# sleep3r/Diffusion-Handwriting-Generation.pytorch

Measured on AMD Instinct MI355X. Metric: stroke-points/sec reverse-sampled (T=60, L=488), higher is better.
Workload: dtype bf16; 1 GPU; configs[1]: batch=64 prompts/GPU, T=60, L=488, Lt=30, d_model=128/192/256, num_layers=2, diffusion_mode=new, random-init weights; global_batch=64, seq_len=488, parallelism=batch-shard x1 (no collectives)

## Files before the change

diffusion-handwriting-generation.pytorch_amd/csrc/attn_core.h:

```cpp
#pragma once
#include "dhw_common.h"

DHW_DEV void frag_keep_keys(Frag<bf16_t>& f, int n0, int n1) {
#pragma unroll
  for (int i = 0; i < 4; ++i) {
    f.v[i] = i < n0 ? f.v[i] : (bf16_t)0.0f;
    f.v[4 + i] = i < n1 ? f.v[4 + i] : (bf16_t)0.0f;
  }
}
DHW_DEV void frag_keep_keys(Frag<float>& f, int n0, int n1) {
#pragma unroll
  for (int i = 0; i < 4; ++i) {
    f.lo[i] = i < n0 ? f.lo[i] : 0.f;
    f.hi[i] = i < n1 ? f.hi[i] : 0.f;
  }
}
template <typename T, int D, int KB>
DHW_DEV void attn_wave16(const Frag<T> (&qf)[(D + 31) / 32], const T* krow, int ldk, const T* vrow, int lpad,
                         const int64_t* trow, int Lk, f32x4 (&o)[D / 16]) {
  constexpr int DT = D / 16, KCH = (D + 31) / 32, NTILE = KB / 16, NPF = KB / 32;
  const int lane = threadIdx.x & 63, g = lane >> 4;
  const float scale = rsqrtf((float)D);
  float m_run = -INFINITY, l_run = 0.f;
#pragma unroll
// ... 126 lines not shown
      const float e = __expf(s[t][r] - m_new);
      s[t][r] = e;
      psum += e;
    }
  l_run = l_run * alpha + psum;
  m_run = m_new;
  Frag<T> pf[NPF];
#pragma unroll
  for (int pp = 0; pp < NPF; ++pp) frag_from_f32(pf[pp], s[2 * pp], s[2 * pp + 1]);
#pragma unroll
  for (int t = 0; t < DT; ++t) {
    o[t] = o[t] * alpha;
#pragma unroll
    for (int pp = 0; pp < NPF; ++pp) {
      const T* vp = reinterpret_cast<const T*>(vt + (16 * t) * SV) + 32 * pp;
      mma32(o[t], frag_load_halves(vp, vp + 16), pf[pp]);
    }
  }
}

typedef __bf16 bf16x4_lds __attribute__((ext_vector_type(4)));
DHW_DEV Frag<bf16_t> frag_load_tr(const char* p0, const char* p1) {
  const bf16x4 a = __builtin_amdgcn_ds_read_tr16_b64_v4bf16((__attribute__((address_space(3))) bf16x4_lds*)(uintptr_t)p0);
  const bf16x4 b = __builtin_amdgcn_ds_read_tr16_b64_v4bf16((__attribute__((address_space(3))) bf16x4_lds*)(uintptr_t)p1);
  Frag<bf16_t> f;
  f.v = __builtin_shufflevector(a, b, 0, 1, 2, 3, 4, 5, 6, 7);
  return f;
}
template <typename T> DHW_DEV void vt_store_piece(char* row, int part, const uint4& v) {
  static_assert(sizeof(T) == 4, "bf16 kernels keep V row-major");
  *reinterpret_cast<uint4*>(row + part * 16) = v;
}

template <int D, int KB, bool MASKED, int NU, bool TAIL>
DHW_DEV void attn_block_bf16(int lane, const Frag<bf16_t> (*qf)[(D + 31) / 32], const char* const (&kt)[NU], int SK, const char* const (&vt)[NU], int SV, int kb,
                             unsigned padbits, int Lk, float (&m_run)[NU], float (&l_run)[NU], f32x4 (*o)[D / 16]) {
#pragma clang fp contract(off)
  typedef bf16_t T;
  constexpr int DT = D / 16, KCH = (D + 31) / 32, NTILE = KB / 16, NPF = KB / 32;
  static_assert(D % 32 == 0, "head width");
  const int g = lane >> 4;
  const float c = rsqrtf((float)D) * 1.4426950408889634f;
  f32x4 s[NU][NTILE];
  {
    Frag<T> kf[NU][NTILE][KCH];
    auto request = [&](int u) {
#pragma unroll
      for (int t = 0; t < NTILE; ++t)
#pragma unroll
        for (int ch = 0; ch < KCH; ++ch) kf[u][t][ch] = frag_load(reinterpret_cast<const T*>(kt[u] + t * 16 * SK) + 32 * ch + 8 * g);
    };
    auto multiply = [&](int u) {
#pragma unroll
      for (int t = 0; t < NTILE; ++t) {
        s[u][t] = (f32x4){0, 0, 0, 0};
#pragma unroll
        for (int ch = 0; ch < KCH; ++ch) mma32(s[u][t], kf[u][t][ch], qf[u][ch]);
      }
    };
    request(0);
#pragma unroll
    for (int u = 0; u < NU; ++u) {
      if (u + 1 < NU) request(u + 1);
      __builtin_amdgcn_sched_barrier(0);
      multiply(u);
      __builtin_amdgcn_sched_barrier(0);
    }
  }
#pragma unroll
  for (int u = 0; u < NU; ++u)
#pragma unroll
    for (int t = 0; t < NTILE; ++t) s[u][t] = s[u][t] * c;
  if constexpr (TAIL) {
#pragma unroll
    for (int u = 0; u < NU; ++u)
#pragma unroll
      for (int t = 0; t < NTILE; ++t)
#pragma unroll
        for (int r = 0; r < 4; ++r) s[u][t][r] = kb + 16 * t + 4 * g + r < Lk ? s[u][t][r] : -INFINITY;
  }
  if constexpr (MASKED) {
    const float neg = -1e9f * 1.4426950408889634f;
#pragma unroll
    for (int u = 0; u < NU; ++u)
#pragma unroll
      for (int t = 0; t < NTILE; ++t)
#pragma unroll
        for (int r = 0; r < 4; ++r) s[u][t][r] += ((padbits >> (4 * t + r)) & 1u) ? neg : 0.f;
  }
  Frag<T> vf[NU][DT][NPF];
#pragma unroll
  for (int u = 0; u < NU; ++u)
#pragma unroll
    for (int t = 0; t < DT; ++t)
#pragma unroll
      for (int pp = 0; pp < NPF; ++pp)
        vf[u][t][pp] = frag_load_tr(vt[u] + 32 * t + (32 * pp) * SV, vt[u] + 32 * t + (32 * pp + 16) * SV);
  __builtin_amdgcn_sched_barrier(0);
  float m_new[NU], alpha[NU];
#pragma unroll
  for (int u = 0; u < NU; ++u) {
    float mx = fmaxf(fmaxf(s[u][0][0], s[u][0][1]), fmaxf(s[u][0][2], s[u][0][3]));
#pragma unroll
    for (int t = 1; t < NTILE; ++t) mx = fmaxf(fmaxf(mx, fmaxf(s[u][t][0], s[u][t][1])), fmaxf(s[u][t][2], s[u][t][3]));
    m_new[u] = fmaxf(m_run[u], xg_max(mx));
    alpha[u] = __builtin_amdgcn_exp2f(m_run[u] - m_new[u]);
    m_run[u] = m_new[u];
  }
  Frag<T> pf[NU][NPF];
#pragma unroll
  for (int u = 0; u < NU; ++u) {
    const f32x4 negm = (f32x4){-m_new[u], -m_new[u], -m_new[u], -m_new[u]};
    f32x4 psum = (f32x4){0, 0, 0, 0};
#pragma unroll
    for (int t = 0; t < NTILE; ++t) {
      s[u][t] = s[u][t] - m_new[u];
#pragma unroll
      for (int r = 0; r < 4; ++r) s[u][t][r] = __builtin_amdgcn_exp2f(s[u][t][r]);
      psum += s[u][t];
    }
    l_run[u] = __builtin_fmaf(l_run[u], alpha[u], (psum[0] + psum[1]) + (psum[2] + psum[3]));
#pragma unroll
    for (int pp = 0; pp < NPF; ++pp) frag_from_f32(pf[u][pp], s[u][2 * pp], s[u][2 * pp + 1]);
  }
  if (kb != 0) {
#pragma unroll
    for (int u = 0; u < NU; ++u)
#pragma unroll
      for (int t = 0; t < DT; ++t) o[u][t] = o[u][t] * alpha[u];
  }
#pragma unroll
  for (int u = 0; u < NU; ++u)
#pragma unroll
    for (int t = 0; t < DT; ++t)
#pragma unroll
      for (int pp = 0; pp < NPF; ++pp) mma32(o[u][t], vf[u][t][pp], pf[u][pp]);
}
template <typename T, int KB, bool MASKED, int UMAX>
DHW_DEV void attn_units(int lane, const Frag<T> (&qf)[UMAX][2], const char* kt, int SK, const char* vt, int SV, int hs, int HS, int H, int kb,
                        unsigned padbits, int Lk, float (&mr)[UMAX], float (&lr)[UMAX], f32x4 (&o)[UMAX][4]) {
  constexpr int ES = sizeof(T);
  const int l15 = lane & 15, g = lane >> 4;
  const char* kt0 = kt + l15 * SK;
  if constexpr (sizeof(T) == 2) {
    const char* vt0 = vt + (4 * g + (l15 >> 2)) * SV + 4 * (l15 & 3) * ES;
#pragma unroll
    for (int u = 0; u < UMAX; ++u) {
      const int h = hs + u * HS;
      if (h < H) {
        const char* const ktu[1] = {kt0 + h * 64 * ES};
        const char* const vtu[1] = {vt0 + h * 64 * ES};
        float m1[1] = {mr[u]}, l1[1] = {lr[u]};
        if (kb + KB > Lk) attn_block_bf16<64, KB, MASKED, 1, true>(lane, qf + u, ktu, SK, vtu, SV, kb, padbits, Lk, m1, l1, o + u);
        else attn_block_bf16<64, KB, MASKED, 1, false>(lane, qf + u, ktu, SK, vtu, SV, kb, padbits, Lk, m1, l1, o + u);
        mr[u] = m1[0]; lr[u] = l1[0];
      }
    }
  } else {
    const char* vt0 = vt + l15 * SV;
#pragma unroll
    for (int u = 0; u < UMAX; ++u) {
      const int h = hs + u * HS;
      if (h < H) attn_block_lds<T, 64, KB>(lane, qf[u], kt0 + h * 64 * ES, SK, vt0 + h * 64 * SV + 4 * g * ES, SV, kb, padbits, Lk, mr[u], lr[u], o[u]);
    }
  }
}

template <int KB>
struct PadMask {
  int64_t tok[KB / 4];
  DHW_DEV void load(int lane, const int64_t* trow, int kb, int Lk) {
    const int g = lane >> 4;
    if (!trow) {
#pragma unroll
      for (int i = 0; i < KB / 4; ++i) tok[i] = 1;
      return;
    }
#pragma unroll
    for (int t = 0; t < KB / 16; ++t)
#pragma unroll
      for (int r = 0; r < 4; ++r) {
        const int key = kb + 16 * t + 4 * g + r;
        tok[4 * t + r] = trow[key < Lk ? key : Lk - 1];
      }
  }
  template <bool LAZY = false>
  DHW_DEV unsigned bits() const {
    unsigned m = 0;
#pragma unroll
    for (int i = 0; i < KB / 4; ++i) {
      int64_t t = tok[i];
      if constexpr (LAZY) asm volatile("" : "+v"(t));
      m |= (t == 0 ? 1u : 0u) << i;
    }
    return m;
  }
// ... 42 lines not shown
```

diffusion-handwriting-generation.pytorch_amd/csrc/enc_a_core.h:

```cpp
#pragma once
#include "attn_core.h"
#include "gemm_core.h"
#include "dhw_kernels.h"

#define ENC_STAMP(slot) do { DHW_STAMP_IF(p.stamps && blockIdx.x == 0 && threadIdx.x == 0, slot, __builtin_amdgcn_s_memrealtime()); \
                             DHW_STAMP_IF(p.stamps && (p.dbg & 4) && blockIdx.x == 0 && (threadIdx.x & 63) == 0, 64 + (threadIdx.x >> 6) * 32 + (slot), __builtin_amdgcn_s_memtime()); } while (0)

template <typename T, int BM>
DHW_DEV void stage_rows(char* dst, int S, const T* src, int C, int b, int L, int m0, int tid, int nthreads) {
  constexpr int ES = sizeof(T);
  const int cpr = C * ES / 16;
  const int total = BM * cpr;
  constexpr int U = 4;
  for (int base = tid; base < total; base += nthreads * U) {
    uint4 v[U];
    int off[U];
#pragma unroll
    for (int u = 0; u < U; ++u) {
      const int id = base + u * nthreads;
      const int r = id / cpr, cc = id - r * cpr;
      v[u] = make_uint4(0, 0, 0, 0);
      off[u] = id < total ? r * S + cc * 16 : -1;
      if (id < total && m0 + r < L)
        v[u] = *reinterpret_cast<const uint4*>(reinterpret_cast<const char*>(src) + ((size_t)(b * L + m0 + r) * C) * ES + (size_t)cc * 16);
    }
#pragma unroll
    for (int u = 0; u < U; ++u)
      if (off[u] >= 0) *reinterpret_cast<uint4*>(dst + off[u]) = v[u];
  }
}

template <int NT>
struct EpiParams {
  f32x4 bias[NT], gam[NT], bet[NT];
  DHW_DEV void load(const float* b, const float* g, const float* be, int n0) {
#pragma unroll
// ... 75 lines not shown
template <typename T, int DM> constexpr int qkv_stride() { return sizeof(T) == 2 ? 3 * DM : 2 * DM; }

template <int DM> constexpr int enc_wn() { return DM % 128 == 0 ? 8 : 6; }

template <typename T, int DM, int BM, int VPIECE = 16, typename P>
DHW_DEV void enc_a_body(const P& p, const EncALds& m, int b, int m0, int rows_valid) {
  constexpr int ES = sizeof(T);
  constexpr int WN = enc_wn<DM>(), WM = 1;
  constexpr int MT = BM / WM / 16, NT = DM / WN / 16, H = DM / 64, KC = DM / 32;
  static_assert(NT * WN * 16 == DM, "channel tiles must divide over the waves");
  const int tid = body_tid(), lane = tid & 63, wave = tid >> 6;
  const int l15 = lane & 15, g = lane >> 4;
  const bool act = WN * WM == 8 || wave < WN * WM;
  const int wm = act ? wave / WN : 0, wn = act ? wave % WN : 0;
  const int S = tile_stride<T>(DM);
  const int Ls = sample_len(p.lens, p.lsh, b, p.Lk);
  char* XR = m.XR;
  char* QR = m.QR;
  float* red = m.red;
  const float* gam = p.film + (size_t)b * p.film_bs;
  const float* bet = gam + p.film_tot;
  const int row0 = wm * (BM / WM), ntile0 = wn * NT;
  const int n0 = ntile0 * 16 + 4 * g;
  const size_t wlane = ((size_t)ntile0 * KC * 64 + lane) * 8;
  const char* xop = XR + (row0 + l15) * S + g * 8 * ES;
  const char* qop = QR + (row0 + l15) * S + g * 8 * ES;

  constexpr int RINGA = sizeof(T) == 4 ? 12 : 24;
  typedef WRing<T, NT, RINGA, (RINGA + NT - 1) / NT> RingT;
  RingT ring;
  constexpr bool SPREADA = sizeof(T) == 2;
  constexpr bool SPREADQ = sizeof(T) == 2 && MT > 1;
  constexpr int FCHA = RingT::template fill_chunks<KC>(), FQA = (FCHA + 3) / 4;
  EpiParams<NT> ep;
  ENC_STAMP(0);
  constexpr bool VROW = sizeof(T) == 2;
  constexpr int KBC = 32, SKC = tile_stride<T>(DM), SVC = VROW ? SKC : KBC * ES + OPAD<T>;
  constexpr int EPV = 16 / ES, CPR = DM / EPV, PPR = KBC / EPV;
  constexpr int UX = (BM * CPR + 511) / 512, UK = (KBC * CPR + 511) / 512, UV = VROW ? UK : (DM * PPR + 511) / 512;
  constexpr int QKS = qkv_stride<T, DM>();
  char* KT = m.KT;
  char* VT = m.VT;
  const T* k1s = reinterpret_cast<const T*>(p.k1) + (size_t)b * p.Lt * DM;
  const T* v1s = reinterpret_cast<const T*>(p.vt1) + (VROW ? (size_t)b * p.Lt * DM : (size_t)b * DM * p.lpadT);
  constexpr bool PLDS = enc_plds<T>();
  const float* PL = m.PL;
  const int64_t* trow = p.text ? p.text + (size_t)b * p.Lt : nullptr;
  PadMask<KBC> pad;
  struct KVRegs { CopyRegs<UK> ck; CopyRegs<UV> cv; };
  auto kv_store = [&](KVRegs& kv) {
    CopyRegs<UK>& ck = kv.ck;
    CopyRegs<UV>& cv = kv.cv;
    ck.store(KBC * CPR, tid, 512, [&](int id) { const int r = id / CPR, cc = id - r * CPR; return reinterpret_cast<uint4*>(KT + r * SKC + cc * 16); },
             [&](int id) { return id / CPR < p.Lt; });
    if constexpr (VROW)
      cv.store(KBC * CPR, tid, 512, [&](int id) { const int r = id / CPR, cc = id - r * CPR; return reinterpret_cast<uint4*>(VT + r * SVC + cc * 16); },
               [&](int id) { return id / CPR < p.Lt; });
    else
      cv.store_to(DM * PPR, tid, 512, [&](int id, const uint4& v) { const int ch = id / PPR, part = id - ch * PPR; vt_store_piece<T>(VT + ch * SVC, part, v); },
                  [&](int id) { return (id % PPR + 1) * EPV <= p.lpadT; });
  };
  {
    KVRegs kv_now;
    KVRegs& kv = [&]() -> KVRegs& { return kv_now; }();
    CopyRegs<UK>& ck = kv.ck;
    CopyRegs<UV>& cv = kv.cv;
// ... 74 lines not shown
      if (kb) {
        attn_stage_kv<T, KBC>(KT, SK, VT, SV, k1s, DM, v1s, VROW ? DM : p.lpadT, DM, kb, p.Lt, tid, 512);
        lds_barrier();
      }
      attn_units<T, KBC, true, UMAX>(lane, qf, KT, SK, VT, SV, hs, HS, H, kb, padbits, p.Lt, mr, lr, o);
      if (kb + KBC < p.Lt) lds_barrier();
    }
#pragma unroll
    for (int u = 0; u < UMAX; ++u) {
      const int h = hs + u * HS;
      float l = lr[u];
      l = xg_sum(l);
      const float inv = 1.0f / l;
      if (h < H) {
        T* dst = reinterpret_cast<T*>(QR + (rg * 16 + l15) * S) + h * 64 + 4 * g;
        store_pair(lane, dst, dst + 16, o[u][0] * inv, o[u][1] * inv);
        store_pair(lane, dst + 32, dst + 48, o[u][2] * inv, o[u][3] * inv);
      }
    }
  }
  if (act) {
    ring.template fill_s<KC>(reinterpret_cast<const T*>(p.w_d1) + wlane);
    if constexpr (!PLDS) ep.load(p.b_d1, gam + p.f1, bet + p.f1, n0);
  }
  lds_barrier();
  ENC_STAMP(3);

  {
    f32x4 acc[NT][MT];
    acc_zero(acc);
    if (act) {
      ring.template run_s<MT, KC>(acc, qop, S, KC);
      ENC_STAMP(10);
      if constexpr (SPREADA) { ring.template fill_begin<KC>(reinterpret_cast<const T*>(p.w_qkv2) + wlane); ring.template fill_range<KC, 0, FQA>(); }
      else ring.template fill_s<KC>(reinterpret_cast<const T*>(p.w_qkv2) + wlane);
      if constexpr (PLDS) ep.lds(PL + DM, PL + 2 * DM, PL + 3 * DM, n0);
#pragma unroll
      for (int i = 0; i < NT; ++i)
#pragma unroll
        for (int j = 0; j < MT; ++j) acc[i][j] += ep.bias[i];
      if constexpr (SPREADA) ring.template fill_range<KC, FQA, 2 * FQA>();
    }
    if constexpr (SPREADA) ln_rows<T, MT, NT, WN, BM>(acc, red, wn, row0, lane, DM, act, [&]() { if (act) ring.template fill_range<KC, 2 * FQA, 3 * FQA>(); });
    else ln_rows<T, MT, NT, WN, BM>(acc, red, wn, row0, lane, DM, act);
    if constexpr (SPREADA) { if (act) ring.template fill_range<KC, 3 * FQA, FCHA>(); }
    ENC_STAMP(11);
    if (act) {
#pragma unroll
      for (int i = 0; i < NT; ++i)
#pragma unroll
        for (int j = 0; j < MT; ++j)
          acc[i][j] = acc[i][j] * ep.gam[i] + ep.bet[i] + load4(reinterpret_cast<const T*>(XR + (row0 + j * 16 + l15) * S) + n0 + 16 * i);
      enc_store_tiles<T, NT, MT>(lane, XR, S, row0, n0, acc);
    }
  }
  lds_barrier();
  ENC_STAMP(4);
  tile_copy_out<T>(XR, S, reinterpret_cast<T*>(p.x2) + (size_t)(b * p.Lk + m0) * DM, DM, rows_valid, DM, tid, 512, DHW_STORE_OF(p.store_a, 1));

  auto qkv_chunk = [&](auto CHUNK_) __attribute__((always_inline)) {
    constexpr int chunk = decltype(CHUNK_)::value;
    int opaque = 0;
    asm volatile("" : "+v"(opaque));
    f32x4 acc[NT][MT];
    acc_zero(acc);
    f32x4 pb[NT][MT];
    const bool rows_out = chunk < 2 || VROW;
    if (act) {
      if constexpr (!PLDS) ep.load_bias(p.b_qkv2 + chunk * DM, n0 + opaque);
      if (chunk < 2) {
#pragma unroll
        for (int i = 0; i < NT; ++i)
#pragma unroll
          for (int j = 0; j < MT; ++j)
            pb[i][j] = *reinterpret_cast<const f32x4*>(p.pb_qk2 + (unsigned)((m0 + row0 + j * 16 + l15) * 2 * DM + chunk * DM + n0 + 16 * i + opaque));
      } else {
#pragma unroll
        for (int i = 0; i < NT; ++i)
#pragma unroll
          for (int j = 0; j < MT; ++j) pb[i][j] = (f32x4){0, 0, 0, 0};
      }
      ring.template run_s<MT, KC>(acc, xop + opaque, S, KC);
      ENC_STAMP(12 + chunk);
      if constexpr (PLDS) ep.lds_bias(PL + (4 + chunk) * DM, n0 + opaque);
      if constexpr (SPREADA && MT == 1) {
        if (chunk < 2) { ring.template fill_begin<KC>(reinterpret_cast<const T*>(p.w_qkv2) + (size_t)(chunk + 1) * DM * DM + wlane); ring.template fill_range<KC, 0, 2 * FQA>(); }
      } else if constexpr (SPREADQ) {
        if (chunk < 2) { ring.template fill_begin<KC>(reinterpret_cast<const T*>(p.w_qkv2) + (size_t)(chunk + 1) * DM * DM + wlane); ring.template fill_range<KC, 0, FQA>(); }
      } else { if (chunk < 2) ring.template fill_s<KC>(reinterpret_cast<const T*>(p.w_qkv2) + (size_t)(chunk + 1) * DM * DM + wlane); }
    }
    if (rows_out && MT == 1) {
      const int r = row0 + l15;
      if (act && r < rows_valid) {
#pragma unroll
        for (int i = 0; i < NT; ++i)
          store4(reinterpret_cast<T*>(p.qk2) + (unsigned)((b * p.Lk + m0 + r) * QKS + chunk * DM + n0 + 16 * i + opaque), acc[i][0] + ep.bias[i] + pb[i][0]);
      }
      if constexpr (SPREADA && MT == 1) { if (act && chunk < 2) ring.template fill_range<KC, 2 * FQA, FCHA>(); }
      ENC_STAMP(5 + chunk);
      return;
    }
    constexpr bool QALT = sizeof(T) == 2;
    char* const QT = QALT && chunk == 1 ? m.KT : QR;
    static_assert(!QALT || (size_t)BM * tile_stride<T>(DM) <= enc_a_text_kv_bytes<T, DM, BM>(), "a staging tile inside the text K / V tiles");
    if constexpr (!QALT) lds_barrier();
    if (rows_out) {
      if (act) {
#pragma unroll
        for (int i = 0; i < NT; ++i)
#pragma unroll
          for (int j = 0; j < MT; ++j) acc[i][j] += ep.bias[i] + pb[i][j];
        if constexpr (SPREADQ) { if (chunk < 2) ring.template fill_range<KC, FQA, 2 * FQA>(); }
        enc_store_tiles<T, NT, MT>(lane, QT, S, row0, n0 + opaque, acc);
        if constexpr (SPREADQ) { if (chunk < 2) ring.template fill_range<KC, 2 * FQA, 3 * FQA>(); }
      }
      lds_barrier();
      tile_copy_out<T>(QT, S, reinterpret_cast<T*>(p.qk2) + (size_t)(b * p.Lk + m0) * QKS + chunk * DM, QKS, rows_valid, DM, tid, 512, DHW_STORE_OF(p.store_a, 1));
      if constexpr (SPREADQ) { if (act && chunk < 2) ring.template fill_range<KC, 3 * FQA, FCHA>(); }
    } else if constexpr (!VROW) {
      constexpr int SV = BM * ES + 16;
      char* VS = m.VS;
      if (act) {
#pragma unroll
        for (int i = 0; i < NT; ++i)
#pragma unroll
          for (int j = 0; j < MT; ++j) {
            const int rl = row0 + j * 16 + l15;
            const f32x4 v = acc[i][j] + ep.bias[i];
#pragma unroll
            for (int k = 0; k < 4; ++k)
              *reinterpret_cast<T*>(VS + (n0 + 16 * i + k) * SV + rl * ES) = from_f<T>(rl < rows_valid ? v[k] : 0.f);
          }
      }
      lds_barrier();
      constexpr int KPP = VPIECE / ES, PPR = BM / KPP;
      const int klimit = m0 + rows_valid >= Ls ? min(BM, p.lpadX - m0) : rows_valid;
      for (int id = tid; id < DM * PPR; id += 512) {
        const int ch = id / PPR, part = id - ch * PPR;
        if ((part + 1) * KPP <= klimit) {
          T* dst = reinterpret_cast<T*>(p.vt2) + ((size_t)b * DM + ch) * p.lpadX + m0 + part * KPP;
          const char* src = VS + ch * SV + part * VPIECE;
          if constexpr (VPIECE == 16) *reinterpret_cast<uint4*>(dst) = *reinterpret_cast<const uint4*>(src);
          else *reinterpret_cast<uint32_t*>(dst) = *reinterpret_cast<const uint32_t*>(src);
        }
      }
    }
    ENC_STAMP(5 + chunk);
  };
  qkv_chunk(std::integral_constant<int, 0>{});
  qkv_chunk(std::integral_constant<int, 1>{});
  qkv_chunk(std::integral_constant<int, 2>{});
// ... 3 lines not shown
```

diffusion-handwriting-generation.pytorch_amd/csrc/enc_bc_core.h:

```cpp
#pragma once
#include "enc_a_core.h"

namespace {

#define STAMP(slot) ENC_STAMP(slot)
#ifdef DHW_STAMPS
#define WST(slot) do { if (p.stamps && blockIdx.x == 0 && lane == 0) p.stamps[64 + wave * 32 + (slot)] = __builtin_amdgcn_s_memtime(); } while (0)
#else
#define WST(slot) do { } while (0)
#endif

template <typename T, int DM, int BM, typename P>
DHW_DEV void enc_a_tile(const P& p, const int b, const int m0, char* smem) {
  const int S = tile_stride<T>(DM);
  EncALds m;
  m.XR = smem;
  m.QR = m.XR + BM * S;
  m.red = reinterpret_cast<float*>(m.QR + BM * S);
  m.KT = reinterpret_cast<char*>(m.red) + 2 * 8 * BM * sizeof(float);
  m.VT = m.KT + 32 * tile_stride<T>(DM);
  m.VS = smem;
  m.PL = reinterpret_cast<float*>(m.KT + enc_a_text_kv_bytes<T, DM, BM>());
  const int Ls = sample_len(p.lens, p.lsh, b, p.Lk);
  if constexpr (DHW_LENS) { if (m0 >= Ls) return; }
  enc_a_body<T, DM, BM>(p, m, b, m0, min(BM, Ls - m0));
}

template <typename T, int DM, int BM>
constexpr size_t self_att_bytes(int kbs, int nbuf, int vpad = 16) {
  return (size_t)BM * tile_stride<T>(DM) + nbuf * ((size_t)kbs * tile_stride<T>(DM) + (sizeof(T) == 2 ? (size_t)kbs * tile_stride<T>(DM) : (size_t)DM * (kbs * sizeof(T) + vpad)));
}
template <typename T, int DM, int BM>
constexpr int self_kbs() { return sizeof(T) == 2 ? 64 : 32; }
template <typename T, int DM, int BM>
// ... 45 lines not shown
  const int row0 = wm * (BM / WM), ntile0 = wn * NT;
  const int n0 = ntile0 * 16 + 4 * g;
  const size_t wlane = ((size_t)ntile0 * KC * 64 + lane) * 8;
  const char* op1 = R1 + (row0 + l15) * S + g * 8 * ES;
  const char* op3 = R3 + (row0 + l15) * S + g * 8 * ES;

  WRing<T, NT, RING, RDMAX> ring;
  constexpr bool SPREAD = sizeof(T) == 2;
  constexpr int FCH = WRing<T, NT, RING, RDMAX>::template fill_chunks<KC>(), FQ = (FCH + 3) / 4;
  EpiParams<NT> ep;
  constexpr bool PLDS = enc_plds<T>(), PLFIX = bc_params_fixed<T, DM, BM>();
  float* PL = reinterpret_cast<float*>(smem + lds_bc_tiles<T, DM, BM>());
  ParamStage<8> cp;
#define BC_PARAMS_REQUEST() cp.template load<DM>(tid, p.b_d2, gam + p.f2, bet + p.f2, p.b_f1, p.b_f1 + DM, p.b_f2, gam + p.f3, bet + p.f3)
  STAMP(16);
  WST(0);
  DHW_STAMP_IF(p.stamps && blockIdx.x == 0 && threadIdx.x == 0, 40, __builtin_amdgcn_s_memtime());
  if (!(p.dbg & 1)) {
    constexpr int RG = BM / 16, HS = 8 / RG, UMAX = (H + HS - 1) / HS, KBS = self_kbs<T, DM, BM>();
    constexpr bool DB = self_db<T, DM, BM>();
    constexpr bool VROW = sizeof(T) == 2;
    constexpr int SK = tile_stride<T>(DM), SV = VROW ? SK : KBS * ES + self_vpad<T, DM, BM>();
    constexpr int BUFB = KBS * SK + (VROW ? KBS * SV : DM * SV);
    constexpr int QKS = qkv_stride<T, DM>();
    const int rg = wave % RG, hs = wave / RG;
    auto unit_head = [&](int u) { return hs + u * HS; };
    const T* qk = reinterpret_cast<const T*>(p.qk2);
    const T* ksrc = qk + (size_t)b * p.Lk * QKS + DM;
    const T* vsrc = VROW ? ksrc + DM : reinterpret_cast<const T*>(p.vt2) + (size_t)b * DM * p.lpadX;
    constexpr int EPV = 16 / ES, CPR = DM / EPV, PPR = KBS / EPV;
    constexpr int UK = (KBS * CPR + 511) / 512, UV = VROW ? UK : (DM * PPR + 511) / 512;
    CopyRegs<UK> ck;
    CopyRegs<UV> cv;
    auto request = [&](int kb) {
      ck.load(KBS * CPR, tid, 512, [&](int id) { const int r = id / CPR, cc = id - r * CPR;
                                                 return reinterpret_cast<const uint4*>(ksrc + (size_t)min(kb + r, p.Lk - 1) * QKS + cc * EPV); });
      if constexpr (VROW)
        cv.load(KBS * CPR, tid, 512, [&](int id) { const int r = id / CPR, cc = id - r * CPR;
                                                   return reinterpret_cast<const uint4*>(vsrc + (size_t)min(kb + r, p.Lk - 1) * QKS + cc * EPV); });
      else
        cv.load(DM * PPR, tid, 512, [&](int id) { const int ch = id / PPR, part = id - ch * PPR;
                                                  return reinterpret_cast<const uint4*>(vsrc + (size_t)ch * p.lpadX + (kb + (part + 1) * EPV <= p.lpadX ? kb + part * EPV : 0)); });
    };
    auto commit = [&](int kb, char* KT, char* VT) {
      ck.store(KBS * CPR, tid, 512, [&](int id) { const int r = id / CPR, cc = id - r * CPR; return reinterpret_cast<uint4*>(KT + r * SK + cc * 16); },
               [&](int id) { return kb + id / CPR < Ls; });
      if constexpr (VROW)
        cv.store(KBS * CPR, tid, 512, [&](int id) { const int r = id / CPR, cc = id - r * CPR; return reinterpret_cast<uint4*>(VT + r * SV + cc * 16); },
                 [&](int id) { return kb + id / CPR < Ls; });
      else
        cv.store_to(DM * PPR, tid, 512, [&](int id, const uint4& v) { const int ch = id / PPR, part = id - ch * PPR; vt_store_piece<T>(VT + ch * SV, part, v); },
                    [&](int id) { return kb + (id % PPR + 1) * EPV <= p.lpadX && (!DHW_LENS || kb + (id % PPR) * EPV < Ls); });
    };
    Frag<T> qf[UMAX][2];
    float mr[UMAX], lr[UMAX];
    f32x4 o[UMAX][4];
#pragma unroll
    for (int u = 0; u < UMAX; ++u) {
      const int h = unit_head(u);
      const T* qrow = qk + (size_t)(b * p.Lk + m0 + rg * 16 + l15) * QKS + (h < H ? h : 0) * 64 + 8 * g;
      qf[u][0] = frag_load(qrow);
      qf[u][1] = frag_load(qrow + 32);
      mr[u] = -INFINITY;
      lr[u] = 0.f;
#pragma unroll
      for (int t = 0; t < 4; ++t) o[u][t] = (f32x4){0, 0, 0, 0};
    }
    if constexpr (PLDS) BC_PARAMS_REQUEST();
    request(0);
    if constexpr (PLDS && PLFIX) cp.template store<DM>(PL, tid);
    commit(0, R2, R2 + KBS * SK);
    lds_barrier();
    int ib = 0;
    auto key_block = [&](int kb) {
      const bool more = kb + KBS < Ls;
      char* KT = R2 + (DB && (ib & 1) ? BUFB : 0);
      char* VT = KT + KBS * SK;
      char* KN = R2 + (DB && !(ib & 1) ? BUFB : 0);
      if (DB && more) request(kb + KBS);
      if (ib < 3) STAMP(26 + 2 * ib);
      attn_units<T, KBS, false, UMAX>(lane, qf, KT, SK, VT, SV, hs, HS, H, kb, 0u, Ls, mr, lr, o);
      if (ib < 3) STAMP(27 + 2 * ib);
      if (more) {
        if (!DB) {
          lds_barrier();
          request(kb + KBS);
        }
        commit(kb + KBS, KN, KN + KBS * SK);
        lds_barrier();
      }
    };
    for (int kb = 0; kb < Ls; kb += KBS, ++ib) key_block(kb);
    if constexpr (PLDS && !PLFIX) {
      static_assert(DB, "a single staging buffer leaves room for a fixed parameter block");
      static_assert((size_t)2 * BM * tile_stride<T>(DM) + 2 * 8 * BM * sizeof(float) + enc_bc_param_bytes<T, DM>() <= (size_t)BUFB, "parameter block inside buffer 0");
      PL = reinterpret_cast<float*>(((ib - 1) & 1) ? R2 + 2 * BM * S + 2 * 8 * BM * sizeof(float) : R2 + BUFB);
      cp.template store<DM>(PL, tid);
    }
    WST(1);
#pragma unroll
    for (int u = 0; u < UMAX; ++u) {
      const int h = unit_head(u);
      float l = lr[u];
      l = xg_sum(l);
      const float inv = 1.0f / l;
      if (h < H) {
        T* dst = reinterpret_cast<T*>(R1 + (rg * 16 + l15) * S) + h * 64 + 4 * g;
        store_pair(lane, dst, dst + 16, o[u][0] * inv, o[u][1] * inv);
        store_pair(lane, dst + 32, dst + 48, o[u][2] * inv, o[u][3] * inv);
      }
    }
  }
  else if constexpr (PLDS) {
    BC_PARAMS_REQUEST();
    if constexpr (!PLFIX) PL = reinterpret_cast<float*>(R2 + 2 * BM * S + 2 * 8 * BM * sizeof(float));
    cp.template store<DM>(PL, tid);
  }
  if (act) {
    ring.template fill_s<KC>(reinterpret_cast<const T*>(p.w_d2) + wlane);
    if constexpr (!PLDS) ep.load(p.b_d2, gam + p.f2, bet + p.f2, n0);
  }
  WST(2);
  lds_barrier();
  WST(3);
  STAMP(17);
// ... 171 lines not shown
```

diffusion-handwriting-generation.pytorch_amd/csrc/gemm_core.h:

```cpp
#pragma once
#include "dhw_common.h"
#include "dhw_kernels.h"
#include "epilogue.h"

template <typename T> constexpr int OPAD = sizeof(T) == 2 ? 32 : 16;
template <typename T> __host__ __device__ constexpr int tile_stride(int C) { return C * (int)sizeof(T) + OPAD<T>; }

DHW_DEV void keep_alive(const Frag<bf16_t>& f) { asm volatile("" ::"v"(f.v)); }
DHW_DEV void keep_alive(const Frag<float>& f) { asm volatile("" ::"v"(f.lo), "v"(f.hi)); }

#ifndef DHW_ABL
#define DHW_ABL 0
#endif
template <typename T, int NT, int RING = (sizeof(T) == 2 ? 24 : 12), int DMAX = 8>
struct WRing {
  static constexpr int D0 = RING / NT;
  static constexpr int D = D0 < 2 ? 2 : (D0 > DMAX ? DMAX : D0);
  Frag<T> q[D][NT];
  const T* base;
  int KT, KTS;

  DHW_DEV void fill(const T* __restrict__ wbase, int kt, int kts = 0) {
    base = wbase;
    KT = kt;
// ... 186 lines not shown
    for (int s = 0; s < KT_; ++s) {
      if (s + PF < KT_) request((s + PF) % NB);
      __builtin_amdgcn_sched_barrier(0);
#pragma unroll
      for (int i = 0; i < NT; ++i)
#pragma unroll
        for (int j = 0; j < MT; ++j) mma32(acc[i][j], q[s][i], a[s % NB][j]);
      if (s < DN) next_chunk(s);
#pragma unroll
      for (int e = 0; e < PER; ++e)
        if (KT_ + s * PER + e < DN) next_chunk(KT_ + s * PER + e);
      __builtin_amdgcn_sched_barrier(0);
    }
    base = nbase; KT = KTN_; KTS = nKTS;
  }
};

template <typename T, int MT, int NT, int RING = (sizeof(T) == 2 ? 24 : 12), int ABL = 0>
DHW_DEV void mainloop(f32x4 (&acc)[NT][MT], const T* __restrict__ wbase, const char* abase, int stride, int KC, int taps,
                      int KTS = 0) {
  WRing<T, NT, RING> ring;
  ring.fill(wbase, KC * taps, KTS);
  ring.template run<MT, ABL>(acc, abase, stride, KC);
}

DHW_DEV __amdgpu_buffer_rsrc_t tile_rsrc(const void* base, unsigned bytes) {
  const unsigned long long a = reinterpret_cast<unsigned long long>(base);
  const unsigned lo = __builtin_amdgcn_readfirstlane((unsigned)a), hi = __builtin_amdgcn_readfirstlane((unsigned)(a >> 32));
  return __builtin_amdgcn_make_buffer_rsrc(reinterpret_cast<void*>(((unsigned long long)hi << 32) | lo), 0, __builtin_amdgcn_readfirstlane(bytes), 0x00020000);
}
DHW_DEV void store16_wt(__amdgpu_buffer_rsrc_t rsrc, unsigned byte_off, const uint4& v) {
  typedef unsigned u32x4_t __attribute__((ext_vector_type(4)));
  __builtin_amdgcn_raw_buffer_store_b128((u32x4_t){v.x, v.y, v.z, v.w}, rsrc, byte_off, 0, 16);
}
DHW_DEV void tile_release_early(int tid) {
  asm volatile("s_waitcnt vmcnt(0)\n\ts_barrier" ::: "memory");
  if (tid == 0) {
    __builtin_amdgcn_fence(__ATOMIC_RELEASE, "agent");
    asm volatile("s_waitcnt vmcnt(0)" ::: "memory");
  }
}

template <typename T>
DHW_DEV void tile_copy_out(const char* lds, int S, T* gdst, int gs, int rows_valid, int C, int tid, int nthreads, int policy = STORE_PLAIN) {
  constexpr int ES = sizeof(T), EPV = 16 / ES;
  const int cpr = C / EPV;
  const int total = rows_valid * cpr;
  if (policy == STORE_WT) {
    if (total <= 0) return;
    const __amdgpu_buffer_rsrc_t rsrc = tile_rsrc(gdst, (unsigned)(((rows_valid - 1) * gs + C) * ES));
    for (int id = tid; id < total; id += nthreads) {
      const int r = id / cpr, cc = id - r * cpr;
      store16_wt(rsrc, (unsigned)((r * gs + cc * EPV) * ES), *reinterpret_cast<const uint4*>(lds + r * S + cc * 16));
    }
    return;
  }
  for (int id = tid; id < total; id += nthreads) {
    const int r = id / cpr, cc = id - r * cpr;
    *reinterpret_cast<uint4*>(gdst + (size_t)r * gs + cc * EPV) = *reinterpret_cast<const uint4*>(lds + r * S + cc * 16);
  }
}
template <typename T>
DHW_DEV void tile_copy_out_pool(const char* lds, int S, T* gdst, int gs, int rows_valid_in, int C, int tid, int nthreads, int policy = STORE_PLAIN) {
  constexpr int ES = sizeof(T), EPV = 16 / ES;
  const int cpr = C / EPV;
  const int total = (rows_valid_in / 2) * cpr;
// ... 118 lines not shown
```

Measured before the change: 1.825 million stroke-points/s.

## Stage bf16 QKV outputs through LDS; add K/V split and reorder variants

By default the bf16 single-M-tile QKV projection no longer writes Q/K/V straight from registers with small scattered stores. It stages them in LDS and uses the cooperative tile copy-out, and the remaining weight-ring prefetch moves after it. Two switch-gated options are added but off by default. One issues the first key block's K and V separately so score computation overlaps the V commit. The other computes QKV chunks in V-K-Q order, with a write-through buffer-store path for a form-1 variant. The aim is more coalesced global stores, at the cost of an extra LDS barrier and copy per chunk.

```diff
diff --git a/diffusion-handwriting-generation.pytorch_amd/csrc/attn_core.h b/diffusion-handwriting-generation.pytorch_amd/csrc/attn_core.h
--- a/diffusion-handwriting-generation.pytorch_amd/csrc/attn_core.h
+++ b/diffusion-handwriting-generation.pytorch_amd/csrc/attn_core.h
@@ -182,12 +182,12 @@
   *reinterpret_cast<uint4*>(row + part * 16) = v;
 }
 
-template <int D, int KB, bool MASKED, int NU, bool TAIL>
-DHW_DEV void attn_block_bf16(int lane, const Frag<bf16_t> (*qf)[(D + 31) / 32], const char* const (&kt)[NU], int SK, const char* const (&vt)[NU], int SV, int kb,
-                             unsigned padbits, int Lk, float (&m_run)[NU], float (&l_run)[NU], f32x4 (*o)[D / 16]) {
+template <int D, int KB, bool MASKED, int NU, bool TAIL, typename VReqF>
+DHW_DEV void attn_scores_bf16(int lane, const Frag<bf16_t> (*qf)[(D + 31) / 32], const char* const (&kt)[NU], int SK, int kb, unsigned padbits, int Lk,
+                              float (&m_run)[NU], float (&l_run)[NU], float (&alpha)[NU], Frag<bf16_t> (&pf)[NU][KB / 32], VReqF vreq) {
 #pragma clang fp contract(off)
   typedef bf16_t T;
-  constexpr int DT = D / 16, KCH = (D + 31) / 32, NTILE = KB / 16, NPF = KB / 32;
+  constexpr int KCH = (D + 31) / 32, NTILE = KB / 16, NPF = KB / 32;
   static_assert(D % 32 == 0, "head width");
   const int g = lane >> 4;
   const float c = rsqrtf((float)D) * 1.4426950408889634f;
@@ -238,16 +238,9 @@
 #pragma unroll
         for (int r = 0; r < 4; ++r) s[u][t][r] += ((padbits >> (4 * t + r)) & 1u) ? neg : 0.f;
   }
-  Frag<T> vf[NU][DT][NPF];
-#pragma unroll
-  for (int u = 0; u < NU; ++u)
-#pragma unroll
-    for (int t = 0; t < DT; ++t)
-#pragma unroll
-      for (int pp = 0; pp < NPF; ++pp)
-        vf[u][t][pp] = frag_load_tr(vt[u] + 32 * t + (32 * pp) * SV, vt[u] + 32 * t + (32 * pp + 16) * SV);
+  vreq();
   __builtin_amdgcn_sched_barrier(0);
-  float m_new[NU], alpha[NU];
+  float m_new[NU];
 #pragma unroll
   for (int u = 0; u < NU; ++u) {
     float mx = fmaxf(fmaxf(s[u][0][0], s[u][0][1]), fmaxf(s[u][0][2], s[u][0][3]));
@@ -257,7 +250,6 @@
     alpha[u] = __builtin_amdgcn_exp2f(m_run[u] - m_new[u]);
     m_run[u] = m_new[u];
   }
-  Frag<T> pf[NU][NPF];
 #pragma unroll
   for (int u = 0; u < NU; ++u) {
     const f32x4 negm = (f32x4){-m_new[u], -m_new[u], -m_new[u], -m_new[u]};
@@ -273,6 +265,18 @@
 #pragma unroll
     for (int pp = 0; pp < NPF; ++pp) frag_from_f32(pf[u][pp], s[u][2 * pp], s[u][2 * pp + 1]);
   }
+}
+template <int D, int KB>
+DHW_DEV void attn_v_request(const char* vt, int SV, Frag<bf16_t> (&vf)[D / 16][KB / 32]) {
+#pragma unroll
+  for (int t = 0; t < D / 16; ++t)
+#pragma unroll
+    for (int pp = 0; pp < KB / 32; ++pp) vf[t][pp] = frag_load_tr(vt + 32 * t + (32 * pp) * SV, vt + 32 * t + (32 * pp + 16) * SV);
+}
+template <int D, int KB, int NU>
+DHW_DEV void attn_pv_bf16(int kb, const float (&alpha)[NU], const Frag<bf16_t> (&pf)[NU][KB / 32], const Frag<bf16_t> (&vf)[NU][D / 16][KB / 32], f32x4 (*o)[D / 16]) {
+#pragma clang fp contract(off)
+  constexpr int DT = D / 16, NPF = KB / 32;
   if (kb != 0) {
 #pragma unroll
     for (int u = 0; u < NU; ++u)
@@ -285,6 +289,18 @@
     for (int t = 0; t < DT; ++t)
 #pragma unroll
       for (int pp = 0; pp < NPF; ++pp) mma32(o[u][t], vf[u][t][pp], pf[u][pp]);
+}
+template <int D, int KB, bool MASKED, int NU, bool TAIL>
+DHW_DEV void attn_block_bf16(int lane, const Frag<bf16_t> (*qf)[(D + 31) / 32], const char* const (&kt)[NU], int SK, const char* const (&vt)[NU], int SV, int kb,
+                             unsigned padbits, int Lk, float (&m_run)[NU], float (&l_run)[NU], f32x4 (*o)[D / 16]) {
+  typedef bf16_t T;
+  Frag<T> vf[NU][D / 16][KB / 32], pf[NU][KB / 32];
+  float alpha[NU];
+  attn_scores_bf16<D, KB, MASKED, NU, TAIL>(lane, qf, kt, SK, kb, padbits, Lk, m_run, l_run, alpha, pf, [&]() {
+#pragma unroll
+    for (int u = 0; u < NU; ++u) attn_v_request<D, KB>(vt[u], SV, vf[u]);
+  });
+  attn_pv_bf16<D, KB, NU>(kb, alpha, pf, vf, o);
 }
 template <typename T, int KB, bool MASKED, int UMAX>
 DHW_DEV void attn_units(int lane, const Frag<T> (&qf)[UMAX][2], const char* kt, int SK, const char* vt, int SV, int hs, int HS, int H, int kb,
@@ -312,6 +328,43 @@
     for (int u = 0; u < UMAX; ++u) {
       const int h = hs + u * HS;
       if (h < H) attn_block_lds<T, 64, KB>(lane, qf[u], kt0 + h * 64 * ES, SK, vt0 + h * 64 * SV + 4 * g * ES, SV, kb, padbits, Lk, mr[u], lr[u], o[u]);
+    }
+  }
+}
+
+template <int KB, int UMAX>
+struct AttnPt {
+  Frag<bf16_t> pf[UMAX][1][KB / 32];
+  float alpha[UMAX][1];
+};
+template <typename T, int KB, bool MASKED, int UMAX>
+DHW_DEV void attn_scores(int lane, const Frag<T> (&qf)[UMAX][2], const char* kt, int SK, int hs, int HS, int H, int kb, unsigned padbits, int Lk,
+                         float (&mr)[UMAX], float (&lr)[UMAX], AttnPt<KB, UMAX>& st) {
+  static_assert(sizeof(T) == 2, "the fp32 parity mode keeps attn_units in one piece");
+  const char* kt0 = kt + (lane & 15) * SK;
+#pragma unroll
+  for (int u = 0; u < UMAX; ++u) {
+    const int h = hs + u * HS;
+    if (h < H) {
+      const char* const ktu[1] = {kt0 + h * 64 * 2};
+      float m1[1] = {mr[u]}, l1[1] = {lr[u]};
+      if (kb + KB > Lk) attn_scores_bf16<64, KB, MASKED, 1, true>(lane, qf + u, ktu, SK, kb, padbits, Lk, m1, l1, st.alpha[u], st.pf[u], []() {});
+      else attn_scores_bf16<64, KB, MASKED, 1, false>(lane, qf + u, ktu, SK, kb, padbits, Lk, m1, l1, st.alpha[u], st.pf[u], []() {});
+      mr[u] = m1[0]; lr[u] = l1[0];
+    }
+  }
+}
+template <int KB, int UMAX>
+DHW_DEV void attn_pv(int lane, const char* vt, int SV, int hs, int HS, int H, int kb, const AttnPt<KB, UMAX>& st, f32x4 (&o)[UMAX][4]) {
+  const int l15 = lane & 15, g = lane >> 4;
+  const char* vt0 = vt + (4 * g + (l15 >> 2)) * SV + 4 * (l15 & 3) * 2;
+#pragma unroll
+  for (int u = 0; u < UMAX; ++u) {
+    const int h = hs + u * HS;
+    if (h < H) {
+      Frag<bf16_t> vf[1][4][KB / 32];
+      attn_v_request<64, KB>(vt0 + h * 64 * 2, SV, vf[0]);
+      attn_pv_bf16<64, KB, 1>(kb, st.alpha[u], st.pf[u], vf, o + u);
     }
   }
 }
diff --git a/diffusion-handwriting-generation.pytorch_amd/csrc/enc_a_core.h b/diffusion-handwriting-generation.pytorch_amd/csrc/enc_a_core.h
--- a/diffusion-handwriting-generation.pytorch_amd/csrc/enc_a_core.h
+++ b/diffusion-handwriting-generation.pytorch_amd/csrc/enc_a_core.h
@@ -2,6 +2,13 @@
 #include "attn_core.h"
 #include "gemm_core.h"
 #include "dhw_kernels.h"
+
+#ifndef DHW_QKV_FORM
+#define DHW_QKV_FORM 2
+#endif
+#ifndef DHW_QKV_VKQ
+#define DHW_QKV_VKQ 0
+#endif
 
 #define ENC_STAMP(slot) do { DHW_STAMP_IF(p.stamps && blockIdx.x == 0 && threadIdx.x == 0, slot, __builtin_amdgcn_s_memrealtime()); \
                              DHW_STAMP_IF(p.stamps && (p.dbg & 4) && blockIdx.x == 0 && (threadIdx.x & 63) == 0, 64 + (threadIdx.x >> 6) * 32 + (slot), __builtin_amdgcn_s_memtime()); } while (0)
@@ -143,6 +150,9 @@
   constexpr bool SPREADA = sizeof(T) == 2;
   constexpr bool SPREADQ = sizeof(T) == 2 && MT > 1;
   constexpr int FCHA = RingT::template fill_chunks<KC>(), FQA = (FCHA + 3) / 4;
+  constexpr int QFORM = sizeof(T) == 2 && MT == 1 ? DHW_QKV_FORM : 0;
+  constexpr bool QVKQ = sizeof(T) == 2 && MT == 1 && DHW_QKV_VKQ;
+  constexpr int QFIRST = QVKQ ? 2 : 0;
   EpiParams<NT> ep;
   ENC_STAMP(0);
   constexpr bool VROW = sizeof(T) == 2;
@@ -283,8 +293,8 @@
     if (act) {
       ring.template run_s<MT, KC>(acc, qop, S, KC);
       ENC_STAMP(10);
-      if constexpr (SPREADA) { ring.template fill_begin<KC>(reinterpret_cast<const T*>(p.w_qkv2) + wlane); ring.template fill_range<KC, 0, FQA>(); }
-      else ring.template fill_s<KC>(reinterpret_cast<const T*>(p.w_qkv2) + wlane);
+      if constexpr (SPREADA) { ring.template fill_begin<KC>(reinterpret_cast<const T*>(p.w_qkv2) + (size_t)QFIRST * DM * DM + wlane); ring.template fill_range<KC, 0, FQA>(); }
+      else ring.template fill_s<KC>(reinterpret_cast<const T*>(p.w_qkv2) + (size_t)QFIRST * DM * DM + wlane);
       if constexpr (PLDS) ep.lds(PL + DM, PL + 2 * DM, PL + 3 * DM, n0);
 #pragma unroll
       for (int i = 0; i < NT; ++i)
@@ -309,8 +319,8 @@
   ENC_STAMP(4);
   tile_copy_out<T>(XR, S, reinterpret_cast<T*>(p.x2) + (size_t)(b * p.Lk + m0) * DM, DM, rows_valid, DM, tid, 512, DHW_STORE_OF(p.store_a, 1));
 
-  auto qkv_chunk = [&](auto CHUNK_) __attribute__((always_inline)) {
-    constexpr int chunk = decltype(CHUNK_)::value;
+  auto qkv_chunk = [&](auto POS_) __attribute__((always_inline)) {
+    constexpr int pos = decltype(POS_)::value, chunk = QVKQ ? 2 - pos : pos, next = QVKQ ? 1 - pos : pos + 1;
     int opaque = 0;
     asm volatile("" : "+v"(opaque));
     f32x4 acc[NT][MT];
@@ -335,19 +345,28 @@
       ENC_STAMP(12 + chunk);
       if constexpr (PLDS) ep.lds_bias(PL + (4 + chunk) * DM, n0 + opaque);
       if constexpr (SPREADA && MT == 1) {
-        if (chunk < 2) { ring.template fill_begin<KC>(reinterpret_cast<const T*>(p.w_qkv2) + (size_t)(chunk + 1) * DM * DM + wlane); ring.template fill_range<KC, 0, 2 * FQA>(); }
+        if (pos < 2) { ring.template fill_begin<KC>(reinterpret_cast<const T*>(p.w_qkv2) + (size_t)next * DM * DM + wlane); ring.template fill_range<KC, 0, 2 * FQA>(); }
       } else if constexpr (SPREADQ) {
-        if (chunk < 2) { ring.template fill_begin<KC>(reinterpret_cast<const T*>(p.w_qkv2) + (size_t)(chunk + 1) * DM * DM + wlane); ring.template fill_range<KC, 0, FQA>(); }
-      } else { if (chunk < 2) ring.template fill_s<KC>(reinterpret_cast<const T*>(p.w_qkv2) + (size_t)(chunk + 1) * DM * DM + wlane); }
-    }
-    if (rows_out && MT == 1) {
+        if (pos < 2) { ring.template fill_begin<KC>(reinterpret_cast<const T*>(p.w_qkv2) + (size_t)next * DM * DM + wlane); ring.template fill_range<KC, 0, FQA>(); }
+      } else { if (pos < 2) ring.template fill_s<KC>(reinterpret_cast<const T*>(p.w_qkv2) + (size_t)next * DM * DM + wlane); }
+    }
+    if (rows_out && MT == 1 && QFORM != 2) {
       const int r = row0 + l15;
-      if (act && r < rows_valid) {
+      if (QFORM == 1 && DHW_STORE_OF(p.store_a, 1) == STORE_WT) {
+        const __amdgpu_buffer_rsrc_t rsrc = tile_rsrc(reinterpret_cast<T*>(p.qk2) + (size_t)(b * p.Lk + m0) * QKS, rows_valid > 0 ? (unsigned)(((rows_valid - 1) * QKS + 3 * DM) * ES) : 0u);
+        if (act) {
+          const unsigned off = (unsigned)((r * QKS + chunk * DM + n0 + opaque) * ES);
+#pragma unroll
+          for (int i = 0; i + 1 < NT; i += 2)
+            store_pair_wt(lane, rsrc, off + 16 * i * ES, off + 16 * (i + 1) * ES, acc[i][0] + ep.bias[i] + pb[i][0], acc[i + 1][0] + ep.bias[i + 1] + pb[i + 1][0], r < rows_valid);
+          if constexpr (NT & 1) { if (r < rows_valid) store8_wt(rsrc, off + 16 * (NT - 1) * ES, pack4_bf16(acc[NT - 1][0] + ep.bias[NT - 1] + pb[NT - 1][0])); }
+        }
+      } else if (act && r < rows_valid) {
 #pragma unroll
         for (int i = 0; i < NT; ++i)
           store4(reinterpret_cast<T*>(p.qk2) + (unsigned)((b * p.Lk + m0 + r) * QKS + chunk * DM + n0 + 16 * i + opaque), acc[i][0] + ep.bias[i] + pb[i][0]);
       }
-      if constexpr (SPREADA && MT == 1) { if (act && chunk < 2) ring.template fill_range<KC, 2 * FQA, FCHA>(); }
+      if constexpr (SPREADA && MT == 1) { if (act && pos < 2) ring.template fill_range<KC, 2 * FQA, FCHA>(); }
       ENC_STAMP(5 + chunk);
       return;
     }
@@ -360,7 +379,10 @@
 #pragma unroll
         for (int i = 0; i < NT; ++i)
 #pragma unroll
-          for (int j = 0; j < MT; ++j) acc[i][j] += ep.bias[i] + pb[i][j];
+          for (int j = 0; j < MT; ++j) {
+            if constexpr (MT == 1) acc[i][j] = acc[i][j] + ep.bias[i] + pb[i][j];
+            else acc[i][j] += ep.bias[i] + pb[i][j];
+          }
         if constexpr (SPREADQ) { if (chunk < 2) ring.template fill_range<KC, FQA, 2 * FQA>(); }
         enc_store_tiles<T, NT, MT>(lane, QT, S, row0, n0 + opaque, acc);
         if constexpr (SPREADQ) { if (chunk < 2) ring.template fill_range<KC, 2 * FQA, 3 * FQA>(); }
@@ -368,6 +390,7 @@
       lds_barrier();
       tile_copy_out<T>(QT, S, reinterpret_cast<T*>(p.qk2) + (size_t)(b * p.Lk + m0) * QKS + chunk * DM, QKS, rows_valid, DM, tid, 512, DHW_STORE_OF(p.store_a, 1));
       if constexpr (SPREADQ) { if (act && chunk < 2) ring.template fill_range<KC, 3 * FQA, FCHA>(); }
+      else if constexpr (SPREADA && MT == 1) { if (act && pos < 2) ring.template fill_range<KC, 2 * FQA, FCHA>(); }
     } else if constexpr (!VROW) {
       constexpr int SV = BM * ES + 16;
       char* VS = m.VS;
diff --git a/diffusion-handwriting-generation.pytorch_amd/csrc/enc_bc_core.h b/diffusion-handwriting-generation.pytorch_amd/csrc/enc_bc_core.h
--- a/diffusion-handwriting-generation.pytorch_amd/csrc/enc_bc_core.h
+++ b/diffusion-handwriting-generation.pytorch_amd/csrc/enc_bc_core.h
@@ -1,5 +1,9 @@
 #pragma once
 #include "enc_a_core.h"
+
+#ifndef DHW_KV_SPLIT
+#define DHW_KV_SPLIT 0
+#endif
 
 namespace {
 
@@ -111,9 +115,11 @@
     constexpr int UK = (KBS * CPR + 511) / 512, UV = VROW ? UK : (DM * PPR + 511) / 512;
     CopyRegs<UK> ck;
     CopyRegs<UV> cv;
-    auto request = [&](int kb) {
+    auto request_k = [&](int kb) {
       ck.load(KBS * CPR, tid, 512, [&](int id) { const int r = id / CPR, cc = id - r * CPR;
                                                  return reinterpret_cast<const uint4*>(ksrc + (size_t)min(kb + r, p.Lk - 1) * QKS + cc * EPV); });
+    };
+    auto request_v = [&](int kb) {
       if constexpr (VROW)
         cv.load(KBS * CPR, tid, 512, [&](int id) { const int r = id / CPR, cc = id - r * CPR;
                                                    return reinterpret_cast<const uint4*>(vsrc + (size_t)min(kb + r, p.Lk - 1) * QKS + cc * EPV); });
@@ -121,9 +127,12 @@
         cv.load(DM * PPR, tid, 512, [&](int id) { const int ch = id / PPR, part = id - ch * PPR;
                                                   return reinterpret_cast<const uint4*>(vsrc + (size_t)ch * p.lpadX + (kb + (part + 1) * EPV <= p.lpadX ? kb + part * EPV : 0)); });
     };
-    auto commit = [&](int kb, char* KT, char* VT) {
+    auto request = [&](int kb) { request_k(kb); request_v(kb); };
+    auto commit_k = [&](int kb, char* KT) {
       ck.store(KBS * CPR, tid, 512, [&](int id) { const int r = id / CPR, cc = id - r * CPR; return reinterpret_cast<uint4*>(KT + r * SK + cc * 16); },
                [&](int id) { return kb + id / CPR < Ls; });
+    };
+    auto commit_v = [&](int kb, char* VT) {
       if constexpr (VROW)
         cv.store(KBS * CPR, tid, 512, [&](int id) { const int r = id / CPR, cc = id - r * CPR; return reinterpret_cast<uint4*>(VT + r * SV + cc * 16); },
                  [&](int id) { return kb + id / CPR < Ls; });
@@ -131,6 +140,7 @@
         cv.store_to(DM * PPR, tid, 512, [&](int id, const uint4& v) { const int ch = id / PPR, part = id - ch * PPR; vt_store_piece<T>(VT + ch * SV, part, v); },
                     [&](int id) { return kb + (id % PPR + 1) * EPV <= p.lpadX && (!DHW_LENS || kb + (id % PPR) * EPV < Ls); });
     };
+    auto commit = [&](int kb, char* KT, char* VT) { commit_k(kb, KT); commit_v(kb, VT); };
     Frag<T> qf[UMAX][2];
     float mr[UMAX], lr[UMAX];
     f32x4 o[UMAX][4];
@@ -146,19 +156,40 @@
       for (int t = 0; t < 4; ++t) o[u][t] = (f32x4){0, 0, 0, 0};
     }
     if constexpr (PLDS) BC_PARAMS_REQUEST();
-    request(0);
+    constexpr bool SPLIT0 = DHW_KV_SPLIT && sizeof(T) == 2;
+    if constexpr (SPLIT0) {
+      __builtin_amdgcn_sched_barrier(0);
+      request_k(0);
+      __builtin_amdgcn_sched_barrier(0);
+      request_v(0);
+      __builtin_amdgcn_sched_barrier(0);
+    } else {
+      request(0);
+    }
     if constexpr (PLDS && PLFIX) cp.template store<DM>(PL, tid);
-    commit(0, R2, R2 + KBS * SK);
+    if constexpr (SPLIT0) commit_k(0, R2);
+    else commit(0, R2, R2 + KBS * SK);
     lds_barrier();
     int ib = 0;
-    auto key_block = [&](int kb) {
+    auto key_block = [&](int kb, auto FIRST_) {
+      constexpr bool first = decltype(FIRST_)::value;
       const bool more = kb + KBS < Ls;
       char* KT = R2 + (DB && (ib & 1) ? BUFB : 0);
       char* VT = KT + KBS * SK;
       char* KN = R2 + (DB && !(ib & 1) ? BUFB : 0);
-      if (DB && more) request(kb + KBS);
+      if (!first && DB && more) request(kb + KBS);
       if (ib < 3) STAMP(26 + 2 * ib);
-      attn_units<T, KBS, false, UMAX>(lane, qf, KT, SK, VT, SV, hs, HS, H, kb, 0u, Ls, mr, lr, o);
+      if constexpr (first) {
+        AttnPt<KBS, UMAX> st;
+        attn_scores<T, KBS, false, UMAX>(lane, qf, KT, SK, hs, HS, H, kb, 0u, Ls, mr, lr, st);
+        __builtin_amdgcn_sched_barrier(0);
+        commit_v(kb, VT);
+        if (DB && more) request(kb + KBS);
+        lds_barrier();
+        attn_pv<KBS, UMAX>(lane, VT, SV, hs, HS, H, kb, st, o);
+      } else {
+        attn_units<T, KBS, false, UMAX>(lane, qf, KT, SK, VT, SV, hs, HS, H, kb, 0u, Ls, mr, lr, o);
+      }
       if (ib < 3) STAMP(27 + 2 * ib);
       if (more) {
         if (!DB) {
@@ -169,7 +200,11 @@
         lds_barrier();
       }
     };
-    for (int kb = 0; kb < Ls; kb += KBS, ++ib) key_block(kb);
+    if constexpr (SPLIT0) {
+      key_block(0, std::true_type{});
+      ib = 1;
+    }
+    for (int kb = SPLIT0 ? KBS : 0; kb < Ls; kb += KBS, ++ib) key_block(kb, std::false_type{});
     if constexpr (PLDS && !PLFIX) {
       static_assert(DB, "a single staging buffer leaves room for a fixed parameter block");
       static_assert((size_t)2 * BM * tile_stride<T>(DM) + 2 * 8 * BM * sizeof(float) + enc_bc_param_bytes<T, DM>() <= (size_t)BUFB, "parameter block inside buffer 0");
diff --git a/diffusion-handwriting-generation.pytorch_amd/csrc/gemm_core.h b/diffusion-handwriting-generation.pytorch_amd/csrc/gemm_core.h
--- a/diffusion-handwriting-generation.pytorch_amd/csrc/gemm_core.h
+++ b/diffusion-handwriting-generation.pytorch_amd/csrc/gemm_core.h
@@ -242,6 +242,17 @@
 DHW_DEV void store16_wt(__amdgpu_buffer_rsrc_t rsrc, unsigned byte_off, const uint4& v) {
   typedef unsigned u32x4_t __attribute__((ext_vector_type(4)));
   __builtin_amdgcn_raw_buffer_store_b128((u32x4_t){v.x, v.y, v.z, v.w}, rsrc, byte_off, 0, 16);
+}
+DHW_DEV void store8_wt(__amdgpu_buffer_rsrc_t rsrc, unsigned byte_off, const uint2& v) {
+  typedef unsigned u32x2_t __attribute__((ext_vector_type(2)));
+  __builtin_amdgcn_raw_buffer_store_b64((u32x2_t){v.x, v.y}, rsrc, byte_off, 0, 16);
+}
+DHW_DEV void store_pair_wt(int lane, __amdgpu_buffer_rsrc_t rsrc, unsigned off0, unsigned off1, const f32x4& v0, const f32x4& v1, bool doit) {
+  const uint2 a = pack4_bf16(v0), b = pack4_bf16(v1);
+  const auto lo = __builtin_amdgcn_permlane16_swap(a.x, b.x, false, false);
+  const auto hi = __builtin_amdgcn_permlane16_swap(a.y, b.y, false, false);
+  const unsigned off = (lane >> 4) & 1 ? off1 - 8 : off0;
+  if (doit) store16_wt(rsrc, off, make_uint4(lo[0], hi[0], lo[1], hi[1]));
 }
 DHW_DEV void tile_release_early(int tid) {
   asm volatile("s_waitcnt vmcnt(0)\n\ts_barrier" ::: "memory");
```

After: 1.834 million stroke-points/s, median of 6. No clear change (+0.5%).
